# annikabrundyn/driving-dirty

Measured on AMD Instinct MI355X. Metric: 6-view scenes/sec fwd+bwd, roadmap model bs=32, higher is better.
Workload: dtype f32

## Files before the change

### driving-dirty_amd/csrc/conv3x3.hip

```cpp
#include <stdlib.h>

#include "dd_common.h"

namespace {

constexpr int EPI_BIAS_RELU_BITS = 5;
constexpr int EPI_RELU_BITS = 6;
constexpr int EPI_BIAS_STATS = 7;
constexpr int EPI_RELU_MASK_AFF = 8;
constexpr int EPI_RELU_BITS_W1 = 9;


template <int CIN, int S>
struct StripCfg {
  static constexpr int PXB = CIN * 4;
  static constexpr int CHUNKS = CIN / 4;
  static constexpr int NPX = 32 * S + 2;
  static constexpr int SLOTB = NPX * PXB;
  static constexpr int NCH = NPX * CHUNKS;
  static constexpr int NLOAD = (NCH + 63) / 64;
  static constexpr int SPILLB = (NLOAD * 64 - NCH) * 16;
  static constexpr int WAVEB = 3 * SLOTB + SPILLB;
  static constexpr int KGROUPS = (CIN == 32) ? 36 : 5;
  static constexpr int WFLOATS = KGROUPS * 64 * 4;
};

template <int CIN>
__device__ __forceinline__ int swz(int q) {
  return CIN == 32 ? ((q >> 1) & 7) : 0;
}

template <int CIN, int S>
__device__ __forceinline__ void load_row(const float* __restrict__ img, int H, int W, int iy, int gx0, int lane,
                                         f32x4 (&r)[StripCfg<CIN, S>::NLOAD]) {
  using C = StripCfg<CIN, S>;
  const bool rowok = (iy >= 0) && (iy < H);
  const __amdgpu_buffer_rsrc_t rs = dd_rsrc(img + (long)(rowok ? iy : 0) * W * CIN, rowok ? W * C::PXB : 0);
#pragma unroll
  for (int i = 0; i < C::NLOAD; ++i) {
    const int c = lane + 64 * i;
    const int q = c / C::CHUNKS, ch = c % C::CHUNKS;
    const int off = (c < C::NCH) ? ((gx0 + q) * C::PXB + ch * 16) : -16;
    r[i] = dd_bload4<DD_AUX_NT>(rs, off);
  }
}

template <int CIN, int S>
__device__ __forceinline__ void load_row_img(const float* __restrict__ img, int H, int W, int iy, int gx0, int lane,
                                             f32x4 (&r)[StripCfg<CIN, S>::NLOAD]) {
  using C = StripCfg<CIN, S>;
  const bool rowok = (iy >= 0) && (iy < H);
  const int so = rowok ? iy * W * C::PXB : 0;
  const __amdgpu_buffer_rsrc_t rs = dd_rsrc(img, rowok ? so + W * C::PXB : 0);
#pragma unroll
  for (int i = 0; i < C::NLOAD; ++i) {
    const int c = lane + 64 * i;
    const int q = c / C::CHUNKS, ch = c % C::CHUNKS;
    const int off = (c < C::NCH) ? ((gx0 + q) * C::PXB + ch * 16) : -16;
    r[i] = dd_bload4<DD_AUX_NT>(rs, off, so);
  }
}

template <int CIN, int S, bool SWZ>
__device__ __forceinline__ void store_row(char* slot, char* spill, int lane,
                                          const f32x4 (&r)[StripCfg<CIN, S>::NLOAD]) {
  using C = StripCfg<CIN, S>;
#pragma unroll
  for (int i = 0; i < C::NLOAD; ++i) {
    const int c = lane + 64 * i;
    const int q = c / C::CHUNKS, ch = c % C::CHUNKS;
    char* dst = slot + q * C::PXB + ((ch ^ (SWZ ? swz<CIN>(q) : 0)) << 4);
    if (64 * (i + 1) > C::NCH) dst = (c < C::NCH) ? dst : spill + (c - C::NCH) * 16;
    *(f32x4*)dst = r[i];
  }
}

template <int S, bool SWZ>
__device__ __forceinline__ void store_row_aff(char* slot, char* spill, int lane, const f32x4 (&r)[StripCfg<32, S>::NLOAD],
                                              bool rowok, int gx0, int W, f32x4 sc, f32x4 sh) {
  using C = StripCfg<32, S>;
#pragma unroll
  for (int i = 0; i < C::NLOAD; ++i) {
    const int c = lane + 64 * i;
    const int q = c / C::CHUNKS, ch = c % C::CHUNKS;
    char* dst = slot + q * C::PXB + ((ch ^ (SWZ ? swz<32>(q) : 0)) << 4);
    if (64 * (i + 1) > C::NCH) dst = (c < C::NCH) ? dst : spill + (c - C::NCH) * 16;
    const bool in = rowok && (gx0 + q >= 0) && (gx0 + q < W);
    f32x4 v = r[i];
    v.x = in ? fmaxf(v.x * sc.x + sh.x, 0.f) : 0.f;
    v.y = in ? fmaxf(v.y * sc.y + sh.y, 0.f) : 0.f;
    v.z = in ? fmaxf(v.z * sc.z + sh.z, 0.f) : 0.f;
    v.w = in ? fmaxf(v.w * sc.w + sh.w, 0.f) : 0.f;
    *(f32x4*)dst = v;
  }
}

template <int CIN, int S, int EPI, int WPB, bool AFF = false>
__global__ __launch_bounds__(WPB * 64) void conv_strip_fwd(const float* __restrict__ x, const float* __restrict__ wp,
                                                           const float* __restrict__ bias,
                                                           const float* __restrict__ msk, float* __restrict__ y,
                                                           unsigned* __restrict__ bits_out, int B, int H, int W, int Ho,
                                                           int Wo, int nstrips, const float* __restrict__ aff = nullptr,
                                                           float* __restrict__ stats = nullptr) {
  using C = StripCfg<CIN, S>;
  extern __shared__ __attribute__((aligned(16))) char smem[];
  const int tid = threadIdx.x;
  const int lane = tid & 63;
  const int wave = __builtin_amdgcn_readfirstlane(tid >> 6);
  {
    f32x4* wl4 = (f32x4*)smem;
    const f32x4* wg4 = (const f32x4*)wp;
    for (int i = tid; i < C::WFLOATS / 4; i += WPB * 64) wl4[i] = wg4[i];
  }
  __syncthreads();
  char* ring = smem + C::WFLOATS * 4 + wave * C::WAVEB;
  char* spill = ring + 3 * C::SLOTB;
  const char* wl = smem;
  const int h = lane >> 5, n = lane & 31;
  const float bv = (EPI == DD_EPI_BIAS || EPI == DD_EPI_BIAS_RELU || EPI == EPI_BIAS_RELU_BITS || EPI == EPI_BIAS_STATS) ? bias[n] : 0.f;
  f32x4 asc = {1.f, 1.f, 1.f, 1.f}, ash = {0.f, 0.f, 0.f, 0.f};
  if (AFF) {
    asc = *(const f32x4*)(aff + 4 * (lane & 7));
    ash = *(const f32x4*)(aff + 32 + 4 * (lane & 7));
  }
  const float msc = (EPI == EPI_RELU_MASK_AFF) ? aff[64 + n] : 1.f, msh = (EPI == EPI_RELU_MASK_AFF) ? aff[96 + n] : 0.f;
  float st_sum = 0.f, st_sq = 0.f;

  long idx, end;
  dd_range((long)B * nstrips * Ho, blockIdx.x * WPB + wave, gridDim.x * WPB, idx, end);
  while (idx < end) {
    const long col = idx / Ho;
    const int y0 = (int)(idx - col * Ho);
    const int y1 = (int)min((long)Ho, y0 + (end - idx));
    idx += y1 - y0;
    const int b = (int)(col / nstrips), x0 = (int)(col % nstrips) * 32;
    const float* xb = x + (long)b * H * W * CIN;
    const int gx0 = S * x0 - 1;

#pragma unroll
    for (int d = 0; d < 3; ++d) {
      f32x4 t[C::NLOAD];
      const int iy = S * y0 - 1 + d;
      load_row<CIN, S>(xb, H, W, iy, gx0, lane, t);
      if constexpr (AFF) store_row_aff<S, true>(ring + ((iy + 1) % 3) * C::SLOTB, spill, lane, t, iy >= 0 && iy < H, gx0, W, asc, ash);
      else store_row<CIN, S, true>(ring + ((iy + 1) % 3) * C::SLOTB, spill, lane, t);
    }

    for (int yy = y0; yy < y1; ++yy) {
      f32x4 pre[S][C::NLOAD];
#pragma unroll
      for (int s = 0; s < S; ++s) load_row<CIN, S>(xb, H, W, S * yy + 2 + s, gx0, lane, pre[s]);

      const long orow = ((long)(b * Ho + yy) * Wo) * 32;
      float mreg[16];
      if (EPI == DD_EPI_RELU_MASK || EPI == EPI_RELU_MASK_AFF) {
        const __amdgpu_buffer_rsrc_t ms = dd_rsrc(msk + orow, Wo * 128);
#pragma unroll
        for (int r = 0; r < 16; ++r) mreg[r] = dd_bload1<DD_AUX_NT>(ms, ((x0 + dd_acc_row(r, lane)) * 32 + n) * 4);
      }
      if (EPI == EPI_RELU_BITS) {
        const __amdgpu_buffer_rsrc_t ms = dd_rsrc((const unsigned*)msk + (long)(b * Ho + yy) * Wo, Wo * 4);
#pragma unroll
        for (int r = 0; r < 16; ++r) mreg[r] = dd_bload1<DD_AUX_NT>(ms, (x0 + dd_acc_row(r, lane)) * 4);
      }
      __builtin_amdgcn_sched_barrier(0);

      f32x16 acc;
#pragma unroll
      for (int r = 0; r < 16; ++r) acc[r] = 0.f;

      if (CIN == 32) {
#pragma unroll
        for (int dy = 0; dy < 3; ++dy) {
          const char* rowb = ring + ((S * yy + dy) % 3) * C::SLOTB;
#pragma unroll
          for (int dx = 0; dx < 3; ++dx) {
            const int q = S * n + dx;
            const char* pa = rowb + q * 128;
            const int sw = swz<32>(q);
#pragma unroll
            for (int j = 0; j < 4; ++j) {
              const f32x4 a = *(const f32x4*)(pa + (((2 * j + h) ^ sw) << 4));
              const f32x4 w = *(const f32x4*)(wl + (((dy * 3 + dx) * 4 + j) * 64 + lane) * 16);
              acc = DD_MFMA(a.x, w.x, acc);
              acc = DD_MFMA(a.y, w.y, acc);
              acc = DD_MFMA(a.z, w.z, acc);
              acc = DD_MFMA(a.w, w.w, acc);
            }
          }
        }
      } else {
#pragma unroll
        for (int jp = 0; jp < 5; ++jp) {
          const int tap = min(2 * jp + h, 8);
          const int dy = tap / 3, dx = tap - 3 * dy;
          const char* rowb = ring + ((S * yy + dy) % 3) * C::SLOTB;
          const f32x4 a = *(const f32x4*)(rowb + (S * n + dx) * 16);
          const f32x4 w = *(const f32x4*)(wl + (jp * 64 + lane) * 16);
          acc = DD_MFMA(a.x, w.x, acc);
          acc = DD_MFMA(a.y, w.y, acc);
          acc = DD_MFMA(a.z, w.z, acc);
        }
      }

#pragma unroll
      for (int s = 0; s < S; ++s) {
        const int iy = S * yy + 2 + s;
        if constexpr (AFF) store_row_aff<S, true>(ring + ((iy + 1) % 3) * C::SLOTB, spill, lane, pre[s], iy >= 0 && iy < H, gx0, W, asc, ash);
        else store_row<CIN, S, true>(ring + ((iy + 1) % 3) * C::SLOTB, spill, lane, pre[s]);
      }

      const __amdgpu_buffer_rsrc_t ys = dd_rsrc(y + orow, Wo * 128);
      unsigned sign_word = 0;
#pragma unroll
      for (int r = 0; r < 16; ++r) {
        float v = acc[r];
        if (EPI == DD_EPI_BIAS || EPI == EPI_BIAS_STATS) v += bv;
        if (EPI == EPI_BIAS_STATS && x0 + dd_acc_row(r, lane) < Wo) {
          st_sum += v;
          st_sq += v * v;
        }
        if (EPI == DD_EPI_BIAS_RELU || EPI == EPI_BIAS_RELU_BITS) v = fmaxf(v + bv, 0.f);
        if (EPI == DD_EPI_RELU_MASK) v = (mreg[r] > 0.f) ? v : 0.f;
        if (EPI == EPI_RELU_MASK_AFF) v = (mreg[r] * msc + msh > 0.f) ? v : 0.f;
        if (EPI == EPI_RELU_BITS) v = ((__builtin_bit_cast(unsigned, mreg[r]) >> n) & 1u) ? v : 0.f;
        dd_bstore1<DD_AUX_NT>(ys, ((x0 + dd_acc_row(r, lane)) * 32 + n) * 4, v);
        if (EPI == EPI_BIAS_RELU_BITS) {
          const unsigned long long m = __ballot(v > 0.f);
          const int i0 = (r & 3) + 8 * (r >> 2);
          if (n == i0) sign_word = (unsigned)m;
          if (n == i0 + 4) sign_word = (unsigned)(m >> 32);
        }
      }
      if (EPI == EPI_BIAS_RELU_BITS) {
        const __amdgpu_buffer_rsrc_t bs = dd_rsrc(bits_out + (long)(b * Ho + yy) * Wo, Wo * 4);
        __builtin_amdgcn_raw_buffer_store_b32(sign_word, bs, (h == 0) ? (x0 + n) * 4 : -16, 0, 0);
      }
    }
  }
  if (EPI == EPI_BIAS_STATS) {
    const long gwl = ((long)(blockIdx.x * WPB + wave) * 64 + lane) * 2;
    stats[gwl] = st_sum;
    stats[gwl + 1] = st_sq;
  }
}

template <int WPB, int MASK>
__global__ __launch_bounds__(WPB * 64) void conv_s2_dgrad(const float* __restrict__ dy, const float* __restrict__ wp,
                                                          const float* __restrict__ msk, float* __restrict__ dx,
                                                          int B, int H, int W, int Ho, int Wo, int nstrips,
                                                          const float* __restrict__ aff = nullptr) {
  using C = StripCfg<32, 1>;
  extern __shared__ __attribute__((aligned(16))) char smem[];
  const int tid = threadIdx.x;
  const int lane = tid & 63;
  const int wave = __builtin_amdgcn_readfirstlane(tid >> 6);
  {
    f32x4* wl4 = (f32x4*)smem;
    const f32x4* wg4 = (const f32x4*)wp;
    for (int i = tid; i < C::WFLOATS / 4; i += WPB * 64) wl4[i] = wg4[i];
  }
  __syncthreads();
  const int nr = (H + 1) / 2;
  const float msc = (MASK == 3) ? aff[64 + (lane & 31)] : 1.f, msh = (MASK == 3) ? aff[96 + (lane & 31)] : 0.f;
  char* ring = smem + C::WFLOATS * 4 + wave * C::WAVEB;
  char* spill = ring + 3 * C::SLOTB;
  const char* wl = smem;
  const int h = lane >> 5, n = lane & 31;

  long idx, end;
  dd_range((long)B * nstrips * nr, blockIdx.x * WPB + wave, gridDim.x * WPB, idx, end);
  while (idx < end) {
    const long col = idx / nr;
    const int r0 = (int)(idx - col * nr);
    const int r1 = (int)min((long)nr, r0 + (end - idx));
    idx += r1 - r0;
    const int b = (int)(col / nstrips), s0 = (int)(col % nstrips) * 32;
    const float* dyb = dy + (long)b * Ho * Wo * 32;

#pragma unroll
    for (int d = 0; d < 2; ++d) {
      f32x4 t[C::NLOAD];
      load_row<32, 1>(dyb, Ho, Wo, r0 + d, s0, lane, t);
      store_row<32, 1, true>(ring + ((r0 + d) % 3) * C::SLOTB, spill, lane, t);
    }

    for (int r = r0; r < r1; ++r) {
      f32x4 pre[C::NLOAD];
      load_row<32, 1>(dyb, Ho, Wo, r + 2, s0, lane, pre);
      __builtin_amdgcn_sched_barrier(0);

      const char* row_r = ring + (r % 3) * C::SLOTB;
      const char* row_r1 = ring + ((r + 1) % 3) * C::SLOTB;
#define DD_TILE(PY, PX, NTAP, ...)                                                              \
  {                                                                                             \
    constexpr int taps[NTAP][3] = {__VA_ARGS__};                                                \
    const int yi = 2 * r + (PY);                                                                \
    const long orow = ((long)(b * H + min(yi, H - 1)) * W) * 32;                                \
    const int obytes = (yi < H) ? W * 128 : 0;                                                  \
    float mreg[16];                                                                             \
    if (MASK == 1 || MASK == 3) {                                                               \
      const __amdgpu_buffer_rsrc_t ms = dd_rsrc(msk + orow, obytes);                            \
      _Pragma("unroll") for (int rr = 0; rr < 16; ++rr)                                         \
        mreg[rr] = dd_bload1<DD_AUX_NT>(ms, ((2 * (s0 + dd_acc_row(rr, lane)) + (PX)) * 32 + n) * 4); \
      __builtin_amdgcn_sched_barrier(0);                                                        \
    }                                                                                           \
    if (MASK == 2) {                                                                            \
      const __amdgpu_buffer_rsrc_t ms = dd_rsrc((const unsigned*)msk + (long)(b * H + min(yi, H - 1)) * W, obytes / 32); \
      _Pragma("unroll") for (int rr = 0; rr < 16; ++rr)                                         \
        mreg[rr] = dd_bload1<DD_AUX_NT>(ms, (2 * (s0 + dd_acc_row(rr, lane)) + (PX)) * 4);      \
      __builtin_amdgcn_sched_barrier(0);                                                        \
    }                                                                                           \
    f32x16 acc;                                                                                 \
    _Pragma("unroll") for (int i = 0; i < 16; ++i) acc[i] = 0.f;                                \
    _Pragma("unroll") for (int t = 0; t < NTAP; ++t) {                                          \
      const char* rowp = taps[t][0] ? row_r1 : row_r;                                           \
      const int q = n + taps[t][1];                                                             \
      const char* pa = rowp + q * 128;                                                          \
      const int sw = swz<32>(q);                                                                \
      _Pragma("unroll") for (int j = 0; j < 4; ++j) {                                           \
        const f32x4 a = *(const f32x4*)(pa + (((2 * j + h) ^ sw) << 4));                        \
        const f32x4 w = *(const f32x4*)(wl + ((taps[t][2] * 4 + j) * 64 + lane) * 16);          \
        acc = DD_MFMA(a.x, w.x, acc);                                                           \
        acc = DD_MFMA(a.y, w.y, acc);                                                           \
        acc = DD_MFMA(a.z, w.z, acc);                                                           \
        acc = DD_MFMA(a.w, w.w, acc);                                                           \
      }                                                                                         \
    }                                                                                           \
    const __amdgpu_buffer_rsrc_t os = dd_rsrc(dx + orow, obytes);                               \
    _Pragma("unroll") for (int rr = 0; rr < 16; ++rr) {                                         \
      float v = acc[rr];                                                                        \
      if (MASK == 1) v = (mreg[rr] > 0.f) ? v : 0.f;                                            \
      if (MASK == 3) v = (mreg[rr] * msc + msh > 0.f) ? v : 0.f;                                \
      if (MASK == 2) v = ((__builtin_bit_cast(unsigned, mreg[rr]) >> n) & 1u) ? v : 0.f;        \
      dd_bstore1<DD_AUX_NT>(os, ((2 * (s0 + dd_acc_row(rr, lane)) + (PX)) * 32 + n) * 4, v);    \
    }                                                                                           \
  }
      DD_TILE(1, 1, 4, {1, 1, 0}, {1, 0, 2}, {0, 1, 6}, {0, 0, 8})
      store_row<32, 1, true>(ring + ((r + 2) % 3) * C::SLOTB, spill, lane, pre);
      DD_TILE(0, 1, 2, {0, 1, 3}, {0, 0, 5})
      DD_TILE(1, 0, 2, {1, 0, 1}, {0, 0, 7})
      DD_TILE(0, 0, 1, {0, 0, 4})
#undef DD_TILE
    }
  }
}

template <int CIN, int S, int WPB, bool AFF = false>
__global__ __launch_bounds__(WPB * 64) void conv_wgrad(const float* __restrict__ x, const float* __restrict__ dy,
                                                       float* __restrict__ part, float* __restrict__ bpart, int B,
                                                       int H, int W, int Ho, int Wo, int nstrips,
                                                       const float* __restrict__ aff = nullptr) {
  using C = StripCfg<CIN, S>;
  constexpr int NT = (CIN == 32) ? 9 : 1;
  extern __shared__ __attribute__((aligned(16))) char smem[];
  const int tid = threadIdx.x;
  const int lane = tid & 63;
  const int wave = __builtin_amdgcn_readfirstlane(tid >> 6);
  char* ring = smem + wave * C::WAVEB;
  char* spill = ring + 3 * C::SLOTB;
  const int h = lane >> 5, n = lane & 31;
  const int gw = blockIdx.x * WPB + wave;
  f32x4 asc = {1.f, 1.f, 1.f, 1.f}, ash = {0.f, 0.f, 0.f, 0.f};
  if (AFF) {
    asc = *(const f32x4*)(aff + 4 * (lane & 7));
    ash = *(const f32x4*)(aff + 32 + 4 * (lane & 7));
  }

  f32x16 acc[NT];
#pragma unroll
  for (int t = 0; t < NT; ++t)
#pragma unroll
    for (int r = 0; r < 16; ++r) acc[t][r] = 0.f;
  float bsum = 0.f;

  const int tap4 = min(n / 3, 8), c4 = n % 3;
  const int dy4 = tap4 / 3, dx4 = tap4 - 3 * dy4;

  long idx, end;
  dd_range((long)B * nstrips * Ho, gw, gridDim.x * WPB, idx, end);
  while (idx < end) {
    const long col = idx / Ho;
    const int y0 = (int)(idx - col * Ho);
    const int y1 = (int)min((long)Ho, y0 + (end - idx));
    idx += y1 - y0;
    const int b = (int)(col / nstrips), x0 = (int)(col % nstrips) * 32;
    const float* xb = x + (long)b * H * W * CIN;
    const float* dyb = dy + (long)b * Ho * Wo * 32;
    const int gx0 = S * x0 - 1;
    const int aoff = ((x0 + h) * 32 + n) * 4;

#pragma unroll
    for (int d = 0; d < 3; ++d) {
      f32x4 t[C::NLOAD];
      const int iy = S * y0 - 1 + d;
      load_row<CIN, S>(xb, H, W, iy, gx0, lane, t);
      if constexpr (AFF) store_row_aff<S, false>(ring + ((iy + 1) % 3) * C::SLOTB, spill, lane, t, iy >= 0 && iy < H, gx0, W, asc, ash);
      else store_row<CIN, S, false>(ring + ((iy + 1) % 3) * C::SLOTB, spill, lane, t);
    }
    float areg[16];
    {
      const __amdgpu_buffer_rsrc_t as = dd_rsrc(dyb + (long)y0 * Wo * 32, Wo * 128);
#pragma unroll
      for (int pp = 0; pp < 16; ++pp) areg[pp] = dd_bload1<DD_AUX_NT>(as, aoff + pp * 256);
    }

    for (int yy = y0; yy < y1; ++yy) {
      f32x4 pre[S][C::NLOAD];
#pragma unroll
      for (int s = 0; s < S; ++s) load_row<CIN, S>(xb, H, W, S * yy + 2 + s, gx0, lane, pre[s]);
      float anext[16];
      {
        const bool ok = yy + 1 < Ho;
        const __amdgpu_buffer_rsrc_t as = dd_rsrc(dyb + (long)(ok ? yy + 1 : 0) * Wo * 32, ok ? Wo * 128 : 0);
#pragma unroll
        for (int pp = 0; pp < 16; ++pp) anext[pp] = dd_bload1<DD_AUX_NT>(as, aoff + pp * 256);
      }
      __builtin_amdgcn_sched_barrier(0);

      if (CIN == 32) {
        const char* rb0 = ring + ((S * yy + 0) % 3) * C::SLOTB;
        const char* rb1 = ring + ((S * yy + 1) % 3) * C::SLOTB;
        const char* rb2 = ring + ((S * yy + 2) % 3) * C::SLOTB;
#pragma unroll
        for (int pp = 0; pp < 16; ++pp) {
          const float a = areg[pp];
          bsum += a;
          const int off = (S * (2 * pp + h)) * 128 + n * 4;
#pragma unroll
          for (int dx = 0; dx < 3; ++dx) {
            acc[0 + dx] = DD_MFMA(a, *(const float*)(rb0 + off + dx * 128), acc[0 + dx]);
            acc[3 + dx] = DD_MFMA(a, *(const float*)(rb1 + off + dx * 128), acc[3 + dx]);
            acc[6 + dx] = DD_MFMA(a, *(const float*)(rb2 + off + dx * 128), acc[6 + dx]);
          }
        }
      } else {
        const char* rb = ring + ((S * yy + dy4) % 3) * C::SLOTB + dx4 * 16 + c4 * 4;
#pragma unroll
        for (int pp = 0; pp < 16; ++pp) {
          const float a = areg[pp];
          bsum += a;
          acc[0] = DD_MFMA(a, *(const float*)(rb + (S * (2 * pp + h)) * 16), acc[0]);
        }
      }

#pragma unroll
      for (int s = 0; s < S; ++s) {
        const int iy = S * yy + 2 + s;
        if constexpr (AFF) store_row_aff<S, false>(ring + ((iy + 1) % 3) * C::SLOTB, spill, lane, pre[s], iy >= 0 && iy < H, gx0, W, asc, ash);
        else store_row<CIN, S, false>(ring + ((iy + 1) % 3) * C::SLOTB, spill, lane, pre[s]);
      }
#pragma unroll
      for (int pp = 0; pp < 16; ++pp) areg[pp] = anext[pp];
    }
  }

#pragma unroll
  for (int t = 0; t < NT; ++t)
#pragma unroll
    for (int r = 0; r < 16; ++r) part[(((long)gw * NT + t) * 16 + r) * 64 + lane] = acc[t][r];
  bpart[(long)gw * 64 + lane] = bsum;
}

template <int CIN>
__global__ __launch_bounds__(1024) void conv_wgrad_reduce(const float* __restrict__ part,
                                                          const float* __restrict__ bpart, float* __restrict__ dw,
                                                          float* __restrict__ db, int nw) {
  constexpr int NT = (CIN == 32) ? 9 : 1;
  constexpr int G = 16;
  __shared__ double red[G][64];
  const int l = threadIdx.x & 63, g = threadIdx.x >> 6;
  const int row = blockIdx.x;
  const float* src = (row < NT * 16) ? part + (long)row * 64 + l : bpart + l;
  const long stride = (row < NT * 16) ? (long)NT * 16 * 64 : 64;
  double s0 = 0.0, s1 = 0.0, s2 = 0.0, s3 = 0.0;
  int w = g;
  for (; w + 3 * G < nw; w += 4 * G) {
    s0 += (double)src[(long)w * stride];
    s1 += (double)src[(long)(w + G) * stride];
    s2 += (double)src[(long)(w + 2 * G) * stride];
    s3 += (double)src[(long)(w + 3 * G) * stride];
  }
  for (; w < nw; w += G) s0 += (double)src[(long)w * stride];
  red[g][l] = (s0 + s1) + (s2 + s3);
  __syncthreads();
  if (g != 0) return;
  double sd = 0.0;
#pragma unroll
  for (int i = 0; i < G; ++i) sd += red[i][l];
  const float s = (float)sd;
  if (row < NT * 16) {
    const int t = row >> 4, r = row & 15;
    const int o = dd_acc_row(r, l), j = l & 31;
    if (CIN == 32) {
      dw[((long)o * 32 + j) * 9 + t] = s;
    } else if (j < 27) {
      dw[((long)o * 3 + (j % 3)) * 9 + (j / 3)] = s;
    }
  } else {
    const double other = __shfl_xor(sd, 32);
    if (l < 32) db[l] = (float)(sd + other);
  }
}

__global__ void conv_pack_kernel(const float* __restrict__ w, float* __restrict__ p, int cin_real, int kind) {
  const int idx = blockIdx.x * blockDim.x + threadIdx.x;
  if (cin_real == 32) {
    if (idx >= 36 * 64 * 4) return;
    const int i = idx & 3, lane = (idx >> 2) & 63, g = idx >> 8;
    const int j = g & 3, t = g >> 2;
    const int n = lane & 31, c = 8 * j + 4 * (lane >> 5) + i;
    float v;
    if (kind == 0) v = w[((long)n * 32 + c) * 9 + t];
    else if (kind == 1) v = w[((long)c * 32 + n) * 9 + (8 - t)];
    else v = w[((long)c * 32 + n) * 9 + t];
    p[idx] = v;
  } else {
    if (idx >= 5 * 64 * 4) return;
    const int i = idx & 3, lane = (idx >> 2) & 63, jp = idx >> 8;
    const int n = lane & 31, tap = 2 * jp + (lane >> 5);
    p[idx] = (tap < 9 && i < 3) ? w[((long)n * 3 + i) * 9 + tap] : 0.f;
  }
}

constexpr int WINO_UFLOATS = 3 * 4 * 2 * 2 * 64 * 4;

__device__ __forceinline__ f32x2 pk_sub2(f32x2 a, f32x2 b) {
  f32x2 r;
  asm("v_pk_add_f32 %0, %1, %2 neg_lo:[0,1] neg_hi:[0,1]" : "=v"(r) : "v"(a), "v"(b));
  return r;
}
__device__ __forceinline__ f32x2 pk_add2(f32x2 a, f32x2 b) {
  f32x2 r;
  asm("v_pk_add_f32 %0, %1, %2" : "=v"(r) : "v"(a), "v"(b));
  return r;
}
__device__ __forceinline__ f32x4 pk_add4a(f32x4 a, f32x4 b) {
  const f32x2 lo = pk_add2(f32x2{a.x, a.y}, f32x2{b.x, b.y}), hi = pk_add2(f32x2{a.z, a.w}, f32x2{b.z, b.w});
  return f32x4{lo.x, lo.y, hi.x, hi.y};
}
__device__ __forceinline__ f32x4 pk_add4(f32x4 a, f32x4 b) {
  const f32x2 lo = f32x2{a.x, a.y} + f32x2{b.x, b.y}, hi = f32x2{a.z, a.w} + f32x2{b.z, b.w};
  return f32x4{lo.x, lo.y, hi.x, hi.y};
}
__device__ __forceinline__ f32x4 pk_sub4(f32x4 a, f32x4 b) {
  f32x2 lo, hi;
  const f32x2 alo = {a.x, a.y}, ahi = {a.z, a.w}, blo = {b.x, b.y}, bhi = {b.z, b.w};
  asm("v_pk_add_f32 %0, %1, %2 neg_lo:[0,1] neg_hi:[0,1]" : "=v"(lo) : "v"(alo), "v"(blo));
  asm("v_pk_add_f32 %0, %1, %2 neg_lo:[0,1] neg_hi:[0,1]" : "=v"(hi) : "v"(ahi), "v"(bhi));
  return f32x4{lo.x, lo.y, hi.x, hi.y};
}

template <int EPI, int WPB>
__global__ __launch_bounds__(WPB * 64) void conv_wino_fwd(const float* __restrict__ x, const float* __restrict__ up,
                                                          const float* __restrict__ bias, const unsigned* __restrict__ bits_in,
                                                          float* __restrict__ y, unsigned* __restrict__ bits_out, int B, int H,
                                                          int W, int nstrips) {
  using C = StripCfg<32, 1>;
  extern __shared__ __attribute__((aligned(16))) char smem[];
  const int tid = threadIdx.x;
  const int lane = tid & 63;
  const int wave = __builtin_amdgcn_readfirstlane(tid >> 6);
  {
    f32x4* ul4 = (f32x4*)smem;
    const f32x4* ug4 = (const f32x4*)up;
    for (int i = tid; i < WINO_UFLOATS / 4; i += WPB * 64) ul4[i] = ug4[i];
  }
  __syncthreads();
  char* ring = smem + WINO_UFLOATS * 4 + wave * C::WAVEB;
  char* spill = ring + 3 * C::SLOTB;
  const f32x4* ul = (const f32x4*)smem;
  const int t16 = lane & 15, q4 = lane >> 4;
  const float bv0 = (EPI == EPI_BIAS_RELU_BITS) ? bias[t16] : 0.f, bv1 = (EPI == EPI_BIAS_RELU_BITS) ? bias[16 + t16] : 0.f;

  long idx, end;
  dd_range((long)B * nstrips * H, blockIdx.x * WPB + wave, gridDim.x * WPB, idx, end);
  while (idx < end) {
    const long col = idx / H;
    const int y0 = (int)(idx - col * H);
    const int y1 = (int)min((long)H, y0 + (end - idx));
    idx += y1 - y0;
    const int b = (int)(col / nstrips), x0 = (int)(col % nstrips) * 32;
    const float* xb = x + (long)b * H * W * 32;
    const int gx0 = x0 - 1;

#pragma unroll
    for (int d = 0; d < 3; ++d) {
      f32x4 t[C::NLOAD];
      const int iy = y0 - 1 + d;
      load_row<32, 1>(xb, H, W, iy, gx0, lane, t);
      store_row<32, 1, true>(ring + ((iy + 1) % 3) * C::SLOTB, spill, lane, t);
    }

    for (int yy = y0; yy < y1; ++yy) {
      f32x4 pre[C::NLOAD];
      load_row<32, 1>(xb, H, W, yy + 2, gx0, lane, pre);
      const long opix = (long)(b * H + yy) * W;
      unsigned mw[8];
      if (EPI == EPI_RELU_BITS) {
        const __amdgpu_buffer_rsrc_t ms = dd_rsrc(bits_in + opix, W * 4);
#pragma unroll
        for (int i = 0; i < 8; ++i)
          mw[i] = __builtin_amdgcn_raw_buffer_load_b32(ms, (x0 + 8 * q4 + i) * 4, 0, 0);
      }
      __builtin_amdgcn_sched_barrier(0);

      f32x4 acc[4][2];
#pragma unroll
      for (int p = 0; p < 4; ++p)
#pragma unroll
        for (int hf = 0; hf < 2; ++hf) acc[p][hf] = f32x4{0.f, 0.f, 0.f, 0.f};

      f32x4 dbuf[2][4], ubuf[2][4][2];
      auto rd = [&](int it, f32x4 (&d)[4], f32x4 (&u)[4][2]) {
        const int ky = it >> 1, g = it & 1;
        const char* rowb = ring + ((yy + ky) % 3) * C::SLOTB;
#pragma unroll
        for (int c = 0; c < 4; ++c) {
          const int px = 2 * t16 + c;
          d[c] = *(const f32x4*)(rowb + px * 128 + (((2 * q4 + g) ^ swz<32>(px)) << 4));
        }
#pragma unroll
        for (int p = 0; p < 4; ++p)
#pragma unroll
          for (int hf = 0; hf < 2; ++hf) u[p][hf] = ul[((((ky * 4 + p) * 2 + hf) * 2 + g) * 64) + lane];
      };
      f32x4 vbuf[2][4];
      auto tf = [&](const f32x4 (&d)[4], f32x4 (&v)[4]) {
        v[0] = pk_sub4(d[0], d[2]);
        v[1] = pk_add4(d[1], d[2]);
        v[2] = pk_sub4(d[2], d[1]);
        v[3] = pk_sub4(d[1], d[3]);
      };
      rd(0, dbuf[0], ubuf[0]);
      tf(dbuf[0], vbuf[0]);
#pragma unroll
      for (int it = 0; it < 6; ++it) {
        if (it + 1 < 6) {
          rd(it + 1, dbuf[(it + 1) & 1], ubuf[(it + 1) & 1]);
          tf(dbuf[(it + 1) & 1], vbuf[(it + 1) & 1]);
        }
        __builtin_amdgcn_sched_barrier(0);
        const f32x4(&u)[4][2] = ubuf[it & 1];
        const f32x4(&v)[4] = vbuf[it & 1];
#pragma unroll
        for (int j = 0; j < 4; ++j)
#pragma unroll
          for (int p = 0; p < 4; ++p)
#pragma unroll
            for (int hf = 0; hf < 2; ++hf) acc[p][hf] = DD_MFMA16(v[p][j], u[p][hf][j], acc[p][hf]);
        __builtin_amdgcn_sched_barrier(0);
      }

      store_row<32, 1, true>(ring + ((yy + 3) % 3) * C::SLOTB, spill, lane, pre);

      const __amdgpu_buffer_rsrc_t ys = dd_rsrc(y + opix * 32, W * 128);
      unsigned keep[8];
#pragma unroll
      for (int i = 0; i < 8; ++i) keep[i] = 0;
#pragma unroll
      for (int r = 0; r < 4; ++r) {
#pragma unroll
        for (int e = 0; e < 2; ++e) {
          const int opx = x0 + 2 * (4 * q4 + r) + e;
          float o[2];
#pragma unroll
          for (int hf = 0; hf < 2; ++hf) {
            const float m0 = acc[0][hf][r], m1 = acc[1][hf][r], m2 = acc[2][hf][r], m3 = acc[3][hf][r];
            float v = e == 0 ? (m0 + m1) + m2 : (m1 - m2) - m3;
            if (EPI == EPI_BIAS_RELU_BITS) v = fmaxf(v + (hf ? bv1 : bv0), 0.f);
            if (EPI == EPI_RELU_BITS) {
              v = ((mw[2 * r + e] >> (t16 + 16 * hf)) & 1u) ? v : 0.f;
            }
            o[hf] = v;
            dd_bstore1<DD_AUX_NT>(ys, (opx * 32 + t16 + 16 * hf) * 4, v);
          }
          if (EPI == EPI_BIAS_RELU_BITS) {
            const unsigned long long b0 = __ballot(o[0] > 0.f), b1 = __ballot(o[1] > 0.f);
            const int G = (lane & 31) >> 3;
            const unsigned w = (unsigned)((b0 >> (16 * G)) & 0xffffull) | ((unsigned)((b1 >> (16 * G)) & 0xffffull) << 16);
            keep[2 * r + e] = w;
          }
        }
      }
      if (EPI == EPI_BIAS_RELU_BITS) {
        const int P = lane & 31, sel = P & 7;
        unsigned word = keep[0];
#pragma unroll
        for (int i = 1; i < 8; ++i) word = (sel == i) ? keep[i] : word;
        const __amdgpu_buffer_rsrc_t bs = dd_rsrc(bits_out + opix, W * 4);
        __builtin_amdgcn_raw_buffer_store_b32(word, bs, (lane < 32) ? (x0 + P) * 4 : -16, 0, 0);
      }
    }
  }
}

constexpr int WINO2_UFLOATS = 16 * 2 * 2 * 64 * 4;

template <int EPI, int WPB>
__global__ __launch_bounds__(WPB * 64) void conv_wino2_fwd(const float* __restrict__ x, const float* __restrict__ up,
                                                           const float* __restrict__ bias, const unsigned* __restrict__ bits_in,
                                                           float* __restrict__ y, unsigned* __restrict__ bits_out, int B, int H,
                                                           int W, int nstrips, const float* __restrict__ x4 = nullptr,
                                                           float* __restrict__ w1part = nullptr) {
  using C = StripCfg<32, 1>;
  using C4 = StripCfg<4, 1>;
  constexpr int RINGB = 4 * C::SLOTB + C::SPILLB;
  constexpr bool W1 = (EPI == EPI_RELU_BITS_W1);
  constexpr bool MASKED = (EPI == EPI_RELU_BITS) || W1;
  extern __shared__ __attribute__((aligned(16))) char smem[];
  const int tid = threadIdx.x;
  const int lane = tid & 63;
  const int wave = __builtin_amdgcn_readfirstlane(tid >> 6);
  {
    f32x4* ul4 = (f32x4*)smem;
    const f32x4* ug4 = (const f32x4*)up;
    for (int i = tid; i < WINO2_UFLOATS / 4; i += WPB * 64) ul4[i] = ug4[i];
  }
  constexpr int W2_XRINGB = 4 * C4::SLOTB + C4::SPILLB;
  constexpr int W2_XBASE = WINO2_UFLOATS * 4 + WPB * RINGB;
  if (W1 && tid < 32) ((float*)(smem + W2_XBASE + WPB * W2_XRINGB))[tid] = 1.f;
  __syncthreads();
  char* xring = smem + W2_XBASE + wave * W2_XRINGB;
  char* xspill = xring + 4 * C4::SLOTB;
  f32x4 wacc[2][2];
#pragma unroll
  for (int hf = 0; hf < 2; ++hf)
#pragma unroll
    for (int nh = 0; nh < 2; ++nh) wacc[hf][nh] = f32x4{0.f, 0.f, 0.f, 0.f};
  char* ring = smem + WINO2_UFLOATS * 4 + wave * RINGB;
  char* spill = ring + 4 * C::SLOTB;
  const f32x4* ul = (const f32x4*)smem;
  const int t16 = lane & 15, q4 = lane >> 4;
  int xky[2], xlane[2];
#pragma unroll
  for (int nh = 0; nh < 2; ++nh) {
    const int c = min(t16 + 16 * nh, 26), tap = c / 3, ci = c - 3 * tap, ky = tap / 3, kx = tap - 3 * ky;
    xky[nh] = ky;
    xlane[nh] = (8 * q4 + kx) * 16 + ci * 4;
  }
  const float bv0 = (EPI == EPI_BIAS_RELU_BITS) ? bias[t16] : 0.f, bv1 = (EPI == EPI_BIAS_RELU_BITS) ? bias[16 + t16] : 0.f;
  const f32x4 bias0 = {bv0, bv0, bv0, bv0}, bias1 = {bv1, bv1, bv1, bv1};
  const int HT = (H + 1) / 2;

  long idx, end;
  dd_range((long)B * nstrips * HT, blockIdx.x * WPB + wave, gridDim.x * WPB, idx, end);
  while (idx < end) {
    const long col = idx / HT;
    const int r0 = (int)(idx - col * HT);
    const int r1 = (int)min((long)HT, r0 + (end - idx));
    idx += r1 - r0;
    const int b = (int)(col / nstrips), x0 = (int)(col % nstrips) * 32;
    const float* xb = x + (long)b * H * W * 32;
    const float* x4b = x4 + (long)b * H * W * 4;
    const int gx0 = x0 - 1;

#pragma unroll
// ... 1586 lines not shown
```

Before: 4285.

## Unroll conv strip row loops by ring phase and software-pipeline LDS reads

The forward and weight-gradient strip kernels now unroll the row loop three ways by ring-buffer phase, so slot offsets become compile-time constants and per-row modulo arithmetic disappears. Row pointers for inputs, outputs and masks advance incrementally instead of being recomputed. LDS fragment reads are issued a few steps ahead of the MFMAs using sched_group_barrier interleaving. For the CIN=32, S=2, 4-wave forward variant, weights are held in registers instead of LDS. The aim is to hide LDS latency and cut address arithmetic, at the cost of higher register pressure and larger code.

```diff
diff --git a/driving-dirty_amd/csrc/conv3x3.hip b/driving-dirty_amd/csrc/conv3x3.hip
--- a/driving-dirty_amd/csrc/conv3x3.hip
+++ b/driving-dirty_amd/csrc/conv3x3.hip
@@ -95,6 +95,36 @@
   }
 }
 
+template <int CIN, int S>
+__device__ __forceinline__ void load_row_at(const float* rowp, bool rowok, int W, int gx0, int lane,
+                                            f32x4 (&r)[StripCfg<CIN, S>::NLOAD]) {
+  using C = StripCfg<CIN, S>;
+  const __amdgpu_buffer_rsrc_t rs = dd_rsrc(rowp, rowok ? W * C::PXB : 0);
+#pragma unroll
+  for (int i = 0; i < C::NLOAD; ++i) {
+    const int c = lane + 64 * i;
+    const int q = c / C::CHUNKS, ch = c % C::CHUNKS;
+    const int off = (c < C::NCH) ? ((gx0 + q) * C::PXB + ch * 16) : -16;
+    r[i] = dd_bload4<DD_AUX_NT>(rs, off);
+  }
+}
+
+__device__ __forceinline__ int dd_row_local(int v) {
+  asm volatile("" : "+v"(v));
+  return v;
+}
+
+template <int P>
+struct Phase {
+  static constexpr int value = P;
+};
+#define DD_ROWS3(S_, PH0, Y0, Y1, row)                                                       \
+  for (int yt_ = (Y0) - ((PH0) * (S_)) % 3; yt_ < (Y1); yt_ += 3) {  \
+    if (yt_ >= (Y0)) row(Phase<0>{}, yt_);                                                   \
+    if (yt_ + 1 >= (Y0) && yt_ + 1 < (Y1)) row(Phase<(S_) % 3>{}, yt_ + 1);                  \
+    if (yt_ + 2 >= (Y0) && yt_ + 2 < (Y1)) row(Phase<(2 * (S_)) % 3>{}, yt_ + 2);            \
+  }
+
 template <int CIN, int S, int EPI, int WPB, bool AFF = false>
 __global__ __launch_bounds__(WPB * 64) void conv_strip_fwd(const float* __restrict__ x, const float* __restrict__ wp,
                                                            const float* __restrict__ bias,
@@ -107,12 +137,18 @@
   const int tid = threadIdx.x;
   const int lane = tid & 63;
   const int wave = __builtin_amdgcn_readfirstlane(tid >> 6);
-  {
+  constexpr bool WREG = (CIN == 32 && S == 2 && WPB == 4);
+  constexpr int NG = C::KGROUPS;
+  f32x4 wreg[WREG ? NG : 1];
+  if constexpr (WREG) {
+#pragma unroll
+    for (int g = 0; g < NG; ++g) wreg[g] = ((const f32x4*)wp)[g * 64 + lane];
+  } else {
     f32x4* wl4 = (f32x4*)smem;
     const f32x4* wg4 = (const f32x4*)wp;
     for (int i = tid; i < C::WFLOATS / 4; i += WPB * 64) wl4[i] = wg4[i];
-  }
-  __syncthreads();
+    __syncthreads();
+  }
   char* ring = smem + C::WFLOATS * 4 + wave * C::WAVEB;
   char* spill = ring + 3 * C::SLOTB;
   const char* wl = smem;
@@ -136,6 +172,7 @@
     const int b = (int)(col / nstrips), x0 = (int)(col % nstrips) * 32;
     const float* xb = x + (long)b * H * W * CIN;
     const int gx0 = S * x0 - 1;
+    const int ph0 = (S * y0) % 3;
 
 #pragma unroll
     for (int d = 0; d < 3; ++d) {
@@ -146,22 +183,34 @@
       else store_row<CIN, S, true>(ring + ((iy + 1) % 3) * C::SLOTB, spill, lane, t);
     }
 
-    for (int yy = y0; yy < y1; ++yy) {
+    const long xpitch = (long)W * CIN;
+    const float* xrow = xb + (S * y0 + 2) * xpitch;
+    const long orow0 = ((long)(b * Ho + y0) * Wo) * 32;
+    float* yrow = y + orow0;
+    const float* mrow = (EPI == DD_EPI_RELU_MASK || EPI == EPI_RELU_MASK_AFF) ? msk + orow0 : nullptr;
+    const unsigned* mbits = (EPI == EPI_RELU_BITS) ? (const unsigned*)msk + (long)(b * Ho + y0) * Wo : nullptr;
+    unsigned* obits = (EPI == EPI_BIAS_RELU_BITS) ? bits_out + (long)(b * Ho + y0) * Wo : nullptr;
+    const int ooff = ((x0 + 4 * h) * 32 + n) * 4;
+    const int boff = (x0 + 4 * h) * 4;
+
+    auto row = [&](auto phase, const int yy) __attribute__((always_inline)) {
+      constexpr int P = decltype(phase)::value;
       f32x4 pre[S][C::NLOAD];
 #pragma unroll
-      for (int s = 0; s < S; ++s) load_row<CIN, S>(xb, H, W, S * yy + 2 + s, gx0, lane, pre[s]);
-
-      const long orow = ((long)(b * Ho + yy) * Wo) * 32;
+      for (int s = 0; s < S; ++s) load_row_at<CIN, S>(xrow + s * xpitch, S * yy + 2 + s < H, W, gx0, lane, pre[s]);
+
       float mreg[16];
       if (EPI == DD_EPI_RELU_MASK || EPI == EPI_RELU_MASK_AFF) {
-        const __amdgpu_buffer_rsrc_t ms = dd_rsrc(msk + orow, Wo * 128);
-#pragma unroll
-        for (int r = 0; r < 16; ++r) mreg[r] = dd_bload1<DD_AUX_NT>(ms, ((x0 + dd_acc_row(r, lane)) * 32 + n) * 4);
+        const __amdgpu_buffer_rsrc_t ms = dd_rsrc(mrow, Wo * 128);
+        const int mo = dd_row_local(ooff);
+#pragma unroll
+        for (int r = 0; r < 16; ++r) mreg[r] = dd_bload1<DD_AUX_NT>(ms, mo + dd_acc_row_half(r, 0) * 128);
       }
       if (EPI == EPI_RELU_BITS) {
-        const __amdgpu_buffer_rsrc_t ms = dd_rsrc((const unsigned*)msk + (long)(b * Ho + yy) * Wo, Wo * 4);
-#pragma unroll
-        for (int r = 0; r < 16; ++r) mreg[r] = dd_bload1<DD_AUX_NT>(ms, (x0 + dd_acc_row(r, lane)) * 4);
+        const __amdgpu_buffer_rsrc_t ms = dd_rsrc(mbits, Wo * 4);
+        const int mo = dd_row_local(boff);
+#pragma unroll
+        for (int r = 0; r < 16; ++r) mreg[r] = dd_bload1<DD_AUX_NT>(ms, mo + dd_acc_row_half(r, 0) * 4);
       }
       __builtin_amdgcn_sched_barrier(0);
 
@@ -169,33 +218,39 @@
 #pragma unroll
       for (int r = 0; r < 16; ++r) acc[r] = 0.f;
 
-      if (CIN == 32) {
-#pragma unroll
-        for (int dy = 0; dy < 3; ++dy) {
-          const char* rowb = ring + ((S * yy + dy) % 3) * C::SLOTB;
-#pragma unroll
-          for (int dx = 0; dx < 3; ++dx) {
-            const int q = S * n + dx;
-            const char* pa = rowb + q * 128;
-            const int sw = swz<32>(q);
-#pragma unroll
-            for (int j = 0; j < 4; ++j) {
-              const f32x4 a = *(const f32x4*)(pa + (((2 * j + h) ^ sw) << 4));
-              const f32x4 w = *(const f32x4*)(wl + (((dy * 3 + dx) * 4 + j) * 64 + lane) * 16);
-              acc = DD_MFMA(a.x, w.x, acc);
-              acc = DD_MFMA(a.y, w.y, acc);
-              acc = DD_MFMA(a.z, w.z, acc);
-              acc = DD_MFMA(a.w, w.w, acc);
-            }
-          }
+      if constexpr (CIN == 32) {
+        constexpr int D = 3;
+        constexpr int RPG = WREG ? 1 : 2;
+        f32x4 a[NG], w[WREG ? 1 : NG];
+        auto request = [&](const int g) __attribute__((always_inline)) {
+          const int dy = g / 12, dx = (g >> 2) % 3, j = g & 3;
+          const int q = S * n + dx;
+          a[g] = *(const f32x4*)(ring + ((P + dy) % 3) * C::SLOTB + q * 128 + (((2 * j + h) ^ swz<32>(q)) << 4));
+          if constexpr (!WREG) w[g] = *(const f32x4*)(wl + (g * 64 + lane) * 16);
+        };
+#pragma unroll
+        for (int g = 0; g < D; ++g) request(g);
+#pragma unroll
+        for (int g = 0; g < NG; ++g) {
+          if (g + D < NG) request(g + D);
+          const f32x4 wv = WREG ? wreg[WREG ? g : 0] : w[WREG ? 0 : g];
+          acc = DD_MFMA(a[g].x, wv.x, acc);
+          acc = DD_MFMA(a[g].y, wv.y, acc);
+          acc = DD_MFMA(a[g].z, wv.z, acc);
+          acc = DD_MFMA(a[g].w, wv.w, acc);
+        }
+        __builtin_amdgcn_sched_group_barrier(0x100, D * RPG, 0);
+#pragma unroll
+        for (int g = 0; g < NG; ++g) {
+          if (g + D < NG) __builtin_amdgcn_sched_group_barrier(0x100, RPG, 0);
+          __builtin_amdgcn_sched_group_barrier(0x008, 4, 0);
         }
       } else {
 #pragma unroll
         for (int jp = 0; jp < 5; ++jp) {
-          const int tap = min(2 * jp + h, 8);
-          const int dy = tap / 3, dx = tap - 3 * dy;
-          const char* rowb = ring + ((S * yy + dy) % 3) * C::SLOTB;
-          const f32x4 a = *(const f32x4*)(rowb + (S * n + dx) * 16);
+          const int t0 = 2 * jp, t1 = (2 * jp + 1 < 8) ? 2 * jp + 1 : 8;
+          const int o0 = ((P + t0 / 3) % 3) * C::SLOTB + (t0 % 3) * 16, o1 = ((P + t1 / 3) % 3) * C::SLOTB + (t1 % 3) * 16;
+          const f32x4 a = *(const f32x4*)(ring + S * n * 16 + (h ? o1 : o0));
           const f32x4 w = *(const f32x4*)(wl + (jp * 64 + lane) * 16);
           acc = DD_MFMA(a.x, w.x, acc);
           acc = DD_MFMA(a.y, w.y, acc);
@@ -205,18 +260,18 @@
 
 #pragma unroll
       for (int s = 0; s < S; ++s) {
-        const int iy = S * yy + 2 + s;
-        if constexpr (AFF) store_row_aff<S, true>(ring + ((iy + 1) % 3) * C::SLOTB, spill, lane, pre[s], iy >= 0 && iy < H, gx0, W, asc, ash);
-        else store_row<CIN, S, true>(ring + ((iy + 1) % 3) * C::SLOTB, spill, lane, pre[s]);
-      }
-
-      const __amdgpu_buffer_rsrc_t ys = dd_rsrc(y + orow, Wo * 128);
+        if constexpr (AFF) store_row_aff<S, true>(ring + ((P + s) % 3) * C::SLOTB, spill, lane, pre[s], S * yy + 2 + s < H, gx0, W, asc, ash);
+        else store_row<CIN, S, true>(ring + ((P + s) % 3) * C::SLOTB, spill, lane, pre[s]);
+      }
+
+      const __amdgpu_buffer_rsrc_t ys = dd_rsrc(yrow, Wo * 128);
+      const int ooff_r = dd_row_local(ooff);
       unsigned sign_word = 0;
 #pragma unroll
       for (int r = 0; r < 16; ++r) {
         float v = acc[r];
         if (EPI == DD_EPI_BIAS || EPI == EPI_BIAS_STATS) v += bv;
-        if (EPI == EPI_BIAS_STATS && x0 + dd_acc_row(r, lane) < Wo) {
+        if (EPI == EPI_BIAS_STATS && x0 + dd_acc_row_half(r, h) < Wo) {
           st_sum += v;
           st_sq += v * v;
         }
@@ -224,7 +279,7 @@
         if (EPI == DD_EPI_RELU_MASK) v = (mreg[r] > 0.f) ? v : 0.f;
         if (EPI == EPI_RELU_MASK_AFF) v = (mreg[r] * msc + msh > 0.f) ? v : 0.f;
         if (EPI == EPI_RELU_BITS) v = ((__builtin_bit_cast(unsigned, mreg[r]) >> n) & 1u) ? v : 0.f;
-        dd_bstore1<DD_AUX_NT>(ys, ((x0 + dd_acc_row(r, lane)) * 32 + n) * 4, v);
+        dd_bstore1<DD_AUX_NT>(ys, ooff_r + dd_acc_row_half(r, 0) * 128, v);
         if (EPI == EPI_BIAS_RELU_BITS) {
           const unsigned long long m = __ballot(v > 0.f);
           const int i0 = (r & 3) + 8 * (r >> 2);
@@ -233,10 +288,16 @@
         }
       }
       if (EPI == EPI_BIAS_RELU_BITS) {
-        const __amdgpu_buffer_rsrc_t bs = dd_rsrc(bits_out + (long)(b * Ho + yy) * Wo, Wo * 4);
+        const __amdgpu_buffer_rsrc_t bs = dd_rsrc(obits, Wo * 4);
         __builtin_amdgcn_raw_buffer_store_b32(sign_word, bs, (h == 0) ? (x0 + n) * 4 : -16, 0, 0);
-      }
-    }
+        obits += Wo;
+      }
+      xrow += S * xpitch;
+      yrow += Wo * 32;
+      if (EPI == DD_EPI_RELU_MASK || EPI == EPI_RELU_MASK_AFF) mrow += Wo * 32;
+      if (EPI == EPI_RELU_BITS) mbits += Wo;
+    };
+    DD_ROWS3(S, ph0, y0, y1, row)
   }
   if (EPI == EPI_BIAS_STATS) {
     const long gwl = ((long)(blockIdx.x * WPB + wave) * 64 + lane) * 2;
@@ -405,54 +466,88 @@
       for (int pp = 0; pp < 16; ++pp) areg[pp] = dd_bload1<DD_AUX_NT>(as, aoff + pp * 256);
     }
 
-    for (int yy = y0; yy < y1; ++yy) {
+    const long xpitch = (long)W * CIN;
+    const float* xrow = xb + (S * y0 + 2) * xpitch;
+    const float* arow = dyb + (long)(y0 + 1) * Wo * 32;
+    const int ph0 = (S * y0) % 3;
+
+    auto row = [&](auto phase, const int yy) __attribute__((always_inline)) {
+      constexpr int P = decltype(phase)::value;
       f32x4 pre[S][C::NLOAD];
 #pragma unroll
-      for (int s = 0; s < S; ++s) load_row<CIN, S>(xb, H, W, S * yy + 2 + s, gx0, lane, pre[s]);
+      for (int s = 0; s < S; ++s) load_row_at<CIN, S>(xrow + s * xpitch, S * yy + 2 + s < H, W, gx0, lane, pre[s]);
       float anext[16];
       {
-        const bool ok = yy + 1 < Ho;
-        const __amdgpu_buffer_rsrc_t as = dd_rsrc(dyb + (long)(ok ? yy + 1 : 0) * Wo * 32, ok ? Wo * 128 : 0);
-#pragma unroll
-        for (int pp = 0; pp < 16; ++pp) anext[pp] = dd_bload1<DD_AUX_NT>(as, aoff + pp * 256);
+        const __amdgpu_buffer_rsrc_t as = dd_rsrc(arow, (yy + 1 < Ho) ? Wo * 128 : 0);
+        const int ao = dd_row_local(aoff);
+#pragma unroll
+        for (int pp = 0; pp < 16; ++pp) anext[pp] = dd_bload1<DD_AUX_NT>(as, ao + pp * 256);
       }
       __builtin_amdgcn_sched_barrier(0);
 
-      if (CIN == 32) {
-        const char* rb0 = ring + ((S * yy + 0) % 3) * C::SLOTB;
-        const char* rb1 = ring + ((S * yy + 1) % 3) * C::SLOTB;
-        const char* rb2 = ring + ((S * yy + 2) % 3) * C::SLOTB;
+      if constexpr (CIN == 32) {
+        constexpr int D = 2;
+        const char* rb = ring + (S * h) * 128 + n * 4;
+        float bx[16][9];
+        auto request = [&](const int pp) __attribute__((always_inline)) {
+#pragma unroll
+          for (int dx = 0; dx < 3; ++dx)
+#pragma unroll
+            for (int dy = 0; dy < 3; ++dy)
+              bx[pp][dy * 3 + dx] = *(const float*)(rb + ((P + dy) % 3) * C::SLOTB + (S * 2 * pp) * 128 + dx * 128);
+        };
+#pragma unroll
+        for (int pp = 0; pp < D; ++pp) request(pp);
 #pragma unroll
         for (int pp = 0; pp < 16; ++pp) {
+          if (pp + D < 16) request(pp + D);
           const float a = areg[pp];
           bsum += a;
-          const int off = (S * (2 * pp + h)) * 128 + n * 4;
 #pragma unroll
           for (int dx = 0; dx < 3; ++dx) {
-            acc[0 + dx] = DD_MFMA(a, *(const float*)(rb0 + off + dx * 128), acc[0 + dx]);
-            acc[3 + dx] = DD_MFMA(a, *(const float*)(rb1 + off + dx * 128), acc[3 + dx]);
-            acc[6 + dx] = DD_MFMA(a, *(const float*)(rb2 + off + dx * 128), acc[6 + dx]);
+            acc[0 + dx] = DD_MFMA(a, bx[pp][0 + dx], acc[0 + dx]);
+            acc[3 + dx] = DD_MFMA(a, bx[pp][3 + dx], acc[3 + dx]);
+            acc[6 + dx] = DD_MFMA(a, bx[pp][6 + dx], acc[6 + dx]);
           }
         }
+        __builtin_amdgcn_sched_group_barrier(0x100, 9 * D, 0);
+#pragma unroll
+        for (int pp = 0; pp < 16; ++pp) {
+          if (pp + D < 16) __builtin_amdgcn_sched_group_barrier(0x100, 9, 0);
+          __builtin_amdgcn_sched_group_barrier(0x008, 9, 0);
+        }
       } else {
-        const char* rb = ring + ((S * yy + dy4) % 3) * C::SLOTB + dx4 * 16 + c4 * 4;
+        constexpr int D = 4;
+        const char* rb = ring + ((P + dy4) % 3) * C::SLOTB + dx4 * 16 + c4 * 4 + (S * h) * 16;
+        float bx[16];
+#pragma unroll
+        for (int pp = 0; pp < D; ++pp) bx[pp] = *(const float*)(rb + (S * 2 * pp) * 16);
 #pragma unroll
         for (int pp = 0; pp < 16; ++pp) {
+          if (pp + D < 16) bx[pp + D] = *(const float*)(rb + (S * 2 * (pp + D)) * 16);
           const float a = areg[pp];
           bsum += a;
-          acc[0] = DD_MFMA(a, *(const float*)(rb + (S * (2 * pp + h)) * 16), acc[0]);
+          acc[0] = DD_MFMA(a, bx[pp], acc[0]);
+        }
+        __builtin_amdgcn_sched_group_barrier(0x100, D, 0);
+#pragma unroll
+        for (int pp = 0; pp < 16; ++pp) {
+          if (pp + D < 16) __builtin_amdgcn_sched_group_barrier(0x100, 1, 0);
+          __builtin_amdgcn_sched_group_barrier(0x008, 1, 0);
         }
       }
 
 #pragma unroll
       for (int s = 0; s < S; ++s) {
-        const int iy = S * yy + 2 + s;
-        if constexpr (AFF) store_row_aff<S, false>(ring + ((iy + 1) % 3) * C::SLOTB, spill, lane, pre[s], iy >= 0 && iy < H, gx0, W, asc, ash);
-        else store_row<CIN, S, false>(ring + ((iy + 1) % 3) * C::SLOTB, spill, lane, pre[s]);
+        if constexpr (AFF) store_row_aff<S, false>(ring + ((P + s) % 3) * C::SLOTB, spill, lane, pre[s], S * yy + 2 + s < H, gx0, W, asc, ash);
+        else store_row<CIN, S, false>(ring + ((P + s) % 3) * C::SLOTB, spill, lane, pre[s]);
       }
 #pragma unroll
       for (int pp = 0; pp < 16; ++pp) areg[pp] = anext[pp];
-    }
+      xrow += S * xpitch;
+      arow += Wo * 32;
+    };
+    DD_ROWS3(S, ph0, y0, y1, row)
   }
 
 #pragma unroll
```

Result: no change. 4321, median of 6 (+0.8%).
